# KieDani/UpliftingTableTennis

Measured on AMD Instinct MI355X. Metric: frames/sec end-to-end (detect+uplift), 1280x720, higher is better.
Workload: dtype bf16

## Files before the change

upliftingtabletennis_amd/csrc/conv.hip:

```cpp
#include "conv_mfma.h"
#include "conv64.h"
#include "conv_stem.h"
#include "conv_bneck.h"
#include "conv_bb.h"
#include "chain16.h"
#include "conv_pointwise.h"

namespace ttup {

int launch_stem(const PackedConv& p1, const PackedConv& p2, const PackedConv& p3, const void* x0, void* t2, void* a1,
                int batch, int h, int w, hipStream_t st, int frames_per_sample) {
    TTUP_REQUIRE((p1.cout == 64 && p1.cin_total == 16 && p1.k == 3 && p1.stride == 1 && p1.ck == 16) ||
                 (p1.cout == 64 && p1.cin_total == 128 && p1.k == 1 && p1.ck == 32), TTUP_EINVAL, "stem: unexpected conv1 shape");
    TTUP_REQUIRE(p2.cout == 64 && p2.cin_total == 64 && p2.k == 3 && p2.stride == 1 && p2.ck == 32, TTUP_EINVAL, "stem: unexpected conv2 shape");
    TTUP_REQUIRE(p3.cout == 32 && p3.cin_total == 64 && p3.k == 1 && p3.ck == 32, TTUP_EINVAL, "stem: unexpected follower shape");
    StemArgs a;
    a.x0 = (const bf16_t*)x0; a.w1 = (const bf16_t*)p1.w_dev; a.b1 = p1.bias_dev; a.w2 = (const bf16_t*)p2.w_dev; a.b2 = p2.bias_dev;
    a.w3 = (const bf16_t*)p3.w_dev; a.b3 = p3.bias_dev; a.t2 = (bf16_t*)t2; a.a1 = (bf16_t*)a1;
    a.H = h; a.W = w; a.tiles_x = cdiv(w, 32); a.tiles_per_img = a.tiles_x * cdiv(h, 8); a.total_tiles = a.tiles_per_img * batch;
    constexpr size_t SMEM = (size_t)(5 * 4 * 64 * 8 + 2 * 9 * 4 * 64 * 8 + 2 * 340 * 32 + 432 * 16) * 2;
    static_assert(SMEM <= 160 * 1024, "LDS budget");
    TTUP_REQUIRE(frames_per_sample == 0 || frames_per_sample == 1 || frames_per_sample == 3, TTUP_EINVAL, "stem: frames per sample must be 0 (X0 records), 1 or 3");
    const bool k4 = p1.k == 1;
    TTUP_REQUIRE(k4 == (frames_per_sample == 3), TTUP_EINVAL, "stem: the 4-step conv1 packing is the three-frame form");
// ... 7 lines not shown
                       void* b0, void* b1, int batch, int h, int w, hipStream_t st) {
    TTUP_REQUIRE(p1.cout == 128 && p1.cin_total == 96 && p1.c0 == 32 && p1.k == 1 && p1.ck == 32, TTUP_EINVAL, "bneck_trans: unexpected conv1 shape");
    TTUP_REQUIRE(p5.cout == 16 && p5.cin_total == 128 && p5.k == 3 && p5.stride == 1 && p5.ck == 32, TTUP_EINVAL, "bneck_trans: unexpected conv5 shape");
    TTUP_REQUIRE(p6.cout == 32 && p6.cin_total == 128 && p6.k == 3 && p6.stride == 2 && p6.ck == 32, TTUP_EINVAL, "bneck_trans: unexpected conv6 shape");
    TTUP_REQUIRE(h % 2 == 0 && w % 2 == 0, TTUP_EINVAL, "bneck_trans: even input size required");
    FusedArgs a;
    a.a2 = (const bf16_t*)a2; a.t2 = (const bf16_t*)t2;
    a.w1 = (const bf16_t*)p1.w_dev; a.b1 = p1.bias_dev; a.w5 = (const bf16_t*)p5.w_dev; a.b5 = p5.bias_dev;
    a.w6 = (const bf16_t*)p6.w_dev; a.b6 = p6.bias_dev; a.b0 = (bf16_t*)b0; a.b1o = (bf16_t*)b1;
    a.H = h; a.W = w; a.tiles_x = cdiv(w, 32); a.tiles_per_img = a.tiles_x * cdiv(h, 8); a.total_tiles = a.tiles_per_img * batch;
    constexpr size_t SMEM = (size_t)(340 * 128 + 3 * 8 * 64 * 8 + 4 * 9 * 64 * 8) * 2 + 512;
    return launch_noted(bneck_trans_kernel, dim3(persistent_grid(a.total_tiles)), 512, SMEM, st, a, "bneck_trans_kernel");
}

constexpr int BB2_TH = 24, BB2_TW = 32;
int bb_chain_tiles_per_img(int h, int w) { return cdiv(w, BB2_TW) * cdiv(h, BB2_TH); }

int launch_bb_chain(const PackedConv* const* convs, int n_convs, const void* x, void* y, int batch, int h, int w,
                    const PackedConv* follow, void* y_follow, hipStream_t st, const BBSum* sum) {
    TTUP_REQUIRE(n_convs == 2 || n_convs == 4, TTUP_EINVAL, "bb_chain: 2 or 4 convs expected");
    const int c = convs[0]->cout;
    BBArgs a;
    a.x = (const bf16_t*)x; a.y = (bf16_t*)y;
    if (sum) {
        TTUP_REQUIRE(c == 16 && n_convs == 4 && sum->n_terms >= 0 && sum->n_terms <= 3, TTUP_EINVAL, "bb_chain: the fused fuse-layer sum rides on the 16-channel two-block chain");
        TTUP_REQUIRE(sum->ysum || (sum->heat && sum->head_w && sum->pv && sum->pi), TTUP_EINVAL, "bb_chain: fused sum needs an output");
        a.nsum = sum->n_terms; a.ysum = (bf16_t*)sum->ysum;
        for (int k = 0; k < sum->n_terms; ++k) { a.st[k] = (const bf16_t*)sum->terms[k]; a.ssh[k] = sum->shifts[k]; }
        a.heat = sum->heat; a.hw = sum->head_w; a.hbias = sum->head_bias; a.pv = sum->pv; a.pi = sum->pi;
    }
    if (follow) {
        TTUP_REQUIRE(c == 32 && n_convs == 2 && follow->cout == 16 && follow->cin_total == 32 && follow->k == 1 && follow->ck == 32 && y_follow, TTUP_EINVAL,
                     "bb_chain: the fused follower is a 1x1 32->16 conv on a 32-channel block");
        a.wf = (const bf16_t*)follow->w_dev; a.bf = follow->bias_dev; a.yf = (bf16_t*)y_follow;
    }
    for (int i = 0; i < n_convs; ++i) {
        const PackedConv& p = *convs[i];
        TTUP_REQUIRE(p.cout == c && p.cin_total == c && p.k == 3 && p.stride == 1 && p.ck == (c == 16 ? 16 : 32), TTUP_EINVAL, "bb_chain: unexpected conv shape");
        a.w[i] = (const bf16_t*)p.w_dev; a.bias[i] = p.bias_dev;
    }
    if (c == 16 && n_convs == 4) {
        static const bool generic = env_set("TTUP_BB2_GENERIC");
        bool shifts_ok = true;
        for (int k = 0; k < a.nsum && k < 3; ++k) shifts_ok = shifts_ok && a.ssh[k] == k + 1;
        const bool sum_stored = !generic && shifts_ok && a.nsum >= 1 && a.nsum <= 3 && a.ysum && !a.heat;
        const bool tail = !generic && shifts_ok && a.nsum == 3 && a.heat && !a.y && !a.ysum;
// ... 54 lines not shown
    std::vector<bf16_t> w((size_t)nchunk * ksteps * mt * 64 * 8);
    size_t idx = 0;
    for (int c = 0; c < nchunk; ++c)
        for (int s = 0; s < ksteps; ++s)
            for (int m = 0; m < mt; ++m)
                for (int l = 0; l < 64; ++l) {
                    const int i = l & 15, g = l >> 4;
                    const int co = (i >> 2) * (4 * mt) + m * 4 + (i & 3);
                    for (int j = 0; j < 8; ++j) {
                        int tap, ci;
                        if (ck == 32) { tap = s; ci = c * 32 + 8 * g + j; }
                        else { tap = 2 * s + (g >> 1); ci = c * 16 + 8 * (g & 1) + j; }
                        w[idx++] = f32_to_bf16(tap < taps ? wval(co, ci, tap) : 0.f);
                    }
                }
    out->ck = ck;
    out->w_bytes = w.size() * sizeof(bf16_t);
    TTUP_HIP_CHECK(hipMalloc(&out->w_dev, out->w_bytes));
    TTUP_HIP_CHECK(hipMemcpy(out->w_dev, w.data(), out->w_bytes, hipMemcpyHostToDevice));
    return TTUP_OK;
}

int launch_conv(const PackedConv& p, const ConvLaunch& l, int dtype, hipStream_t st) {
    if (dtype == TTUP_DTYPE_F32) {
        TTUP_REQUIRE(!l.res2 && !l.res3, TTUP_EINVAL, "conv: extra fuse-layer terms are a bf16-path fusion");
        static const bool direct = env_set("TTUP_F32_DIRECT");
        static const bool exact = env_set("TTUP_F32_EXACT");
        if (!direct && !exact && conv_x3_supported(p)) return launch_conv_x3(p, l, st);
        if (!direct && conv_f32_mfma_supported(p)) return launch_conv_f32_mfma(p, l, st);
        TTUP_REQUIRE(!l.n_active, TTUP_EINVAL, "conv: a device-side batch needs the matrix-pipe fp32 kernel");
        ConvFArgs a;
        a.src0 = (const float*)l.src0; a.src1 = (const float*)l.src1; a.w = (const float*)p.w_dev; a.bias = p.bias_dev;
        a.residual = (const float*)l.residual; a.dst = (float*)l.dst;
        a.c0 = p.c0; a.c1 = p.cin_total - p.c0; a.cout = p.cout; a.ks = p.k; a.stride = p.stride;
        a.H = l.h; a.W = l.w; a.OH = (l.h + p.stride - 1) / p.stride; a.OW = (l.w + p.stride - 1) / p.stride; a.relu = l.relu;
        a.total = (long long)l.batch * a.OH * a.OW * a.cout;
        const int threads = 256;
        const long long blocks = (a.total + threads - 1) / threads;
        kernel_note("conv_direct_f32_kernel");
        hipLaunchKernelGGL(conv_direct_f32_kernel, dim3((unsigned)blocks), dim3(threads), 0, st, a);
        TTUP_LAUNCH_CHECK();
        return TTUP_OK;
    }
    TTUP_REQUIRE(!(l.res2 || l.res3) || (p.stride == 2 && !l.follow), TTUP_EINVAL, "conv: extra fuse-layer terms ride on the stride-2 chain convs only");
    if (l.follow) {
        TTUP_REQUIRE(p.k == 3 && p.stride == 1 && p.ck == 32 && p.cout == 64, TTUP_EINVAL, "conv: fused follower needs a 3x3 s1 conv with 64 outputs");
// ... 112 lines not shown
```

upliftingtabletennis_amd/csrc/conv64.h:

```cpp
#pragma once
#include "conv_mfma.h"

namespace ttup {

struct NoHook { __device__ __forceinline__ void operator()(int) const {} };
template <int NPIX = 340, typename Hook = NoHook>
__device__ __forceinline__ void conv64_tile_mfma(f32x4 (&acc)[4][2], const bf16_t* const (&bB)[3], const bf16_t* s_w, int wave, int lane, Hook hook = Hook()) {
    constexpr int IW = 34;
    bf16x8 brow[2][4], af[2][4];
    auto load_b = [&](bf16x8 (&br)[4], int c, int dx) __attribute__((always_inline)) {
#pragma unroll
        for (int rr = 0; rr < 4; ++rr) br[rr] = *(const bf16x8*)(bB[dx] + c * (NPIX * 32) + ((2 * (wave >> 1) + rr) * IW + (wave & 1) * 16) * 32);
    };
    auto load_a = [&](bf16x8 (&a4)[4], int st) __attribute__((always_inline)) {
#pragma unroll
        for (int m = 0; m < 4; ++m) a4[m] = *(const bf16x8*)(s_w + ((st * 4 + m) * 64 + lane) * 8);
    };
    load_b(brow[0], 0, 0);
    load_a(af[0], 0);
#pragma unroll
    for (int s = 0; s < 18; ++s) {
        const int dy = s % 3, gi = s / 3;
        if (s + 1 < 18) {
            const int s1 = s + 1, dy1 = s1 % 3, g1 = s1 / 3, c1 = g1 / 3, dx1 = g1 % 3;
// ... 113 lines not shown
#pragma unroll
                for (int r = 0; r < 4; ++r) v[m * 4 + r] = acc[m][t][r];
            if (a.residual) {
#pragma unroll
                for (int q = 0; q < 2; ++q) {
                    const u32x4 rv = rres[t][q];
                    const unsigned w4[4] = {rv.x, rv.y, rv.z, rv.w};
#pragma unroll
                    for (int k = 0; k < 4; ++k) { v[q * 8 + 2 * k] += bf16_to_f32((bf16_t)(w4[k] & 0xffff)); v[q * 8 + 2 * k + 1] += bf16_to_f32((bf16_t)(w4[k] >> 16)); }
                }
            }
#pragma unroll
            for (int q = 0; q < 2; ++q)
#pragma unroll
                for (int i = 0; i < 4; ++i) { const unsigned w = pack2(v[q * 8 + 2 * i], v[q * 8 + 2 * i + 1]); pk[t][q][i] = a.relu ? relu_pk(w) : w; }
        }
#pragma unroll
        for (int t = 0; t < 2; ++t) {
            const int oy = oy0 + 2 * (wave >> 1) + t, ox = ox0 + (wave & 1) * 16 + n;
            const bool ok = oy < a.H && ox < a.W;
            if (!(L16 || L32) && !ok) continue;
            const size_t opix = ok ? (size_t)(b * a.H + oy) * a.W + ox : 0;
            const size_t o = opix * 64 + g * 16;
#pragma unroll
            for (int q = 0; q < 2; ++q)
                if (ok) *(u32x4*)(a.dst + o + q * 8) = pk[t][q];
            if (L16) {
                f32x4 c = bl16;
#pragma unroll
                for (int k = 0; k < 2; ++k) c = __builtin_amdgcn_mfma_f32_16x16x32_bf16(al16[k], __builtin_bit_cast(bf16x8, pk[t][k]), c, 0, 0, 0);
                if (ok) *(u32x2*)(a.dl16 + opix * 16 + g * 4) = u32x2{pack2(c[0], c[1]), pack2(c[2], c[3])};
            }
            if (L32) {
                f32x4 c[2] = {bl32[0], bl32[1]};
#pragma unroll
                for (int k = 0; k < 2; ++k)
#pragma unroll
                    for (int m = 0; m < 2; ++m) c[m] = __builtin_amdgcn_mfma_f32_16x16x32_bf16(al32[k][m], __builtin_bit_cast(bf16x8, pk[t][k]), c[m], 0, 0, 0);
                if (ok) *(u32x4*)(a.dl32 + opix * 32 + g * 8) = u32x4{pack2(c[0][0], c[0][1]), pack2(c[0][2], c[0][3]), pack2(c[1][0], c[1][1]), pack2(c[1][2], c[1][3])};
            }
        }
    }
}

template <bool L16, bool L32>
__global__ __launch_bounds__(512) void conv64_dma_kernel(ConvKArgs a) {
    constexpr int IH = 10, IW = 34, NPIX = IH * IW;
    constexpr int W_U = 2 * 9 * 4 * 64;
    constexpr int IN_UNITS = NPIX * 8, IN_PT = (IN_UNITS + 511) / 512;
// ... 87 lines not shown
#pragma unroll
                for (int r = 0; r < 4; ++r) v[m * 4 + r] = acc[m][t][r];
            if (a.residual) {
#pragma unroll
                for (int q = 0; q < 2; ++q) {
                    const u32x4 rv = rres[t][q];
                    const unsigned w4[4] = {rv.x, rv.y, rv.z, rv.w};
#pragma unroll
                    for (int k = 0; k < 4; ++k) { v[q * 8 + 2 * k] += bf16_to_f32((bf16_t)(w4[k] & 0xffff)); v[q * 8 + 2 * k + 1] += bf16_to_f32((bf16_t)(w4[k] >> 16)); }
                }
            }
#pragma unroll
            for (int q = 0; q < 2; ++q)
#pragma unroll
                for (int i = 0; i < 4; ++i) { const unsigned w = pack2(v[q * 8 + 2 * i], v[q * 8 + 2 * i + 1]); pk[t][q][i] = a.relu ? relu_pk(w) : w; }
        }
#pragma unroll
        for (int t = 0; t < 2; ++t) {
            const int oy = oy0 + 2 * (wave >> 1) + t, ox = ox0 + (wave & 1) * 16 + n;
            const bool ok = oy < a.H && ox < a.W;
            if (!(L16 || L32) && !ok) continue;
            const size_t opix = ok ? (size_t)(b * a.H + oy) * a.W + ox : 0;
            const size_t o = opix * 64 + g * 16;
#pragma unroll
            for (int q = 0; q < 2; ++q)
                if (ok) *(u32x4*)(a.dst + o + q * 8) = pk[t][q];
            if (L16) {
                f32x4 c = bl16;
#pragma unroll
                for (int k = 0; k < 2; ++k) c = __builtin_amdgcn_mfma_f32_16x16x32_bf16(al16[k], __builtin_bit_cast(bf16x8, pk[t][k]), c, 0, 0, 0);
                if (ok) *(u32x2*)(a.dl16 + opix * 16 + g * 4) = u32x2{pack2(c[0], c[1]), pack2(c[2], c[3])};
            }
            if (L32) {
                f32x4 c[2] = {bl32[0], bl32[1]};
#pragma unroll
                for (int k = 0; k < 2; ++k)
#pragma unroll
                    for (int m = 0; m < 2; ++m) c[m] = __builtin_amdgcn_mfma_f32_16x16x32_bf16(al32[k][m], __builtin_bit_cast(bf16x8, pk[t][k]), c[m], 0, 0, 0);
                if (ok) *(u32x4*)(a.dl32 + opix * 32 + g * 8) = u32x4{pack2(c[0][0], c[0][1]), pack2(c[0][2], c[0][3]), pack2(c[1][0], c[1][1]), pack2(c[1][2], c[1][3])};
            }
        }
    };
    f32x4 acc[4][2];
    u32x4 rres[2][2] = {};
    for (int it = 0; it < my_tiles; ++it) {
        const TileAt tile = tile_at<8, 32>(xcd_tile(blockIdx.x + it * gridDim.x, a.total_tiles), a.tiles_per_img, a.tiles_x);
        const int b = tile.b, oy0 = tile.y0, ox0 = tile.x0;
        __syncthreads();
        if (a.residual) {
// ... 18 lines not shown
        epilogue(acc, rres, b, oy0, ox0);
    }
}

template <bool DMA, bool L16, bool L32>
static int launch_conv64_t(const ConvKArgs& a, hipStream_t st) {
    constexpr size_t SMEM = (size_t)(2 * 9 * 4 * 64 * 8 + (DMA ? 2 : 1) * 2 * 340 * 32) * 2;
    return launch_noted(DMA ? conv64_dma_kernel<L16, L32> : conv64_kernel<L16, L32>, dim3(persistent_grid(a.total_tiles)), 512, SMEM, st, a,
                        DMA ? "conv64_dma_kernel<%s, %s>" : "conv64_kernel<%s, %s>", L16 ? "true" : "false", L32 ? "true" : "false");
}
template <bool DMA>
static int launch_conv64_followers(const ConvKArgs& a, hipStream_t st) {
    if (a.dl16 && a.dl32) return launch_conv64_t<DMA, true, true>(a, st);
    if (a.dl16) return launch_conv64_t<DMA, true, false>(a, st);
    if (a.dl32) return launch_conv64_t<DMA, false, true>(a, st);
    return launch_conv64_t<DMA, false, false>(a, st);
}

static int launch_conv64(const PackedConv& p, const ConvLaunch& l, hipStream_t st) {
    ConvKArgs a;
    a.src0 = (const bf16_t*)l.src0; a.wpack = (const bf16_t*)p.w_dev; a.bias = p.bias_dev; a.residual = (const bf16_t*)l.residual; a.dst = (bf16_t*)l.dst;
    a.H = l.h; a.W = l.w; a.OH = l.h; a.OW = l.w; a.relu = l.relu;
    a.tiles_x = cdiv(l.w, 32); a.tiles_per_img = a.tiles_x * cdiv(l.h, 8); a.total_tiles = a.tiles_per_img * l.batch;
    if (l.lin16) {
        TTUP_REQUIRE(l.lin16->cout == 16 && l.lin16->cin_total == 64 && l.lin16->k == 1 && l.lin16->ck == 32 && l.lin16_dst, TTUP_EINVAL, "conv64: bad 64->16 follower");
        a.wl16 = (const bf16_t*)l.lin16->w_dev; a.bl16 = l.lin16->bias_dev; a.dl16 = (bf16_t*)l.lin16_dst;
    }
    if (l.lin32) {
        TTUP_REQUIRE(l.lin32->cout == 32 && l.lin32->cin_total == 64 && l.lin32->k == 1 && l.lin32->ck == 32 && l.lin32_dst, TTUP_EINVAL, "conv64: bad 64->32 follower");
        a.wl32 = (const bf16_t*)l.lin32->w_dev; a.bl32 = l.lin32->bias_dev; a.dl32 = (bf16_t*)l.lin32_dst;
    }
    static const bool dma = env_ll("TTUP_CONV64_DMA", 1) != 0;
    return dma ? launch_conv64_followers<true>(a, st) : launch_conv64_followers<false>(a, st);
}

}
```

upliftingtabletennis_amd/csrc/conv_mfma.h:

```cpp
#pragma once
#include "conv_dev.h"
#include "conv.h"

namespace ttup {

struct ConvKArgs {
    const bf16_t* src0 = nullptr;
    const bf16_t* src1 = nullptr;
    const bf16_t* wpack = nullptr;
    const float* bias = nullptr;
    const bf16_t* residual = nullptr;
    bf16_t* dst = nullptr;
    int c0 = 0, c1 = 0;
    int nchunk0 = 0, nchunk = 0;
    int H = 0, W = 0, OH = 0, OW = 0;
    int tiles_x = 0, tiles_per_img = 0, total_tiles = 0;
    int relu = 0;
    const bf16_t* w11 = nullptr; const float* bias11 = nullptr; bf16_t* dst11 = nullptr;
    const bf16_t* res2 = nullptr; const bf16_t* res3 = nullptr; int sh3 = 0;
    const bf16_t* wl16 = nullptr; const float* bl16 = nullptr; bf16_t* dl16 = nullptr;
    const bf16_t* wl32 = nullptr; const float* bl32 = nullptr; bf16_t* dl32 = nullptr;
    const bf16_t* wpack_b = nullptr; const float* bias_b = nullptr; bf16_t* dst_b = nullptr; int relu_b = 0;
    int xcd = 0;
};
// ... 211 lines not shown
                    *(u32x4*)(s_t + p * 64 + (((2 * g + q) ^ (p & 7)) << 3)) = pk;
                }
            }
            __syncthreads();
#pragma unroll
            for (int t = 0; t < NT; ++t) {
                const int nt = wave * NT + t;
                const int p = (nt / NTW) * TW + (nt % NTW) * 16 + n;
                f32x4 c11[2] = {bias11[0], bias11[1]};
#pragma unroll
                for (int k = 0; k < 2; ++k) {
                    const bf16x8 bfr = *(const bf16x8*)(s_t + p * 64 + (((4 * k + g) ^ (p & 7)) << 3));
#pragma unroll
                    for (int m = 0; m < 2; ++m) c11[m] = __builtin_amdgcn_mfma_f32_16x16x32_bf16(af11[k][m], bfr, c11[m], 0, 0, 0);
                }
                const int oy = oy0 + nt / NTW, ox = ox0 + (nt % NTW) * 16 + n;
                if (oy >= a.OH || ox >= a.OW) continue;
                *(u32x4*)(a.dst11 + ((size_t)(b * a.OH + oy) * a.OW + ox) * 32 + g * 8) = pack8(c11[0], c11[1], true);
            }
        }
    }
}

__global__ __launch_bounds__(512) void conv_s2_pair_kernel(ConvKArgs a) {
    constexpr int CK = 16, KS = 3, S = 2, TH = 4, TW = 32, MTA = 2, MTB = 1;
    constexpr int IH = (TH - 1) * S + KS, IW = (TW - 1) * S + KS;
    constexpr int KSTEPS = 5, PAD = 1;
    constexpr int IN_ELEMS = IH * IW * CK;
    constexpr int IN_UNITS = IH * IW * (CK / 8), IN_PT = (IN_UNITS + 511) / 512;
    constexpr int WA_UNITS = KSTEPS * MTA * 64, WB_UNITS = KSTEPS * MTB * 64;
    extern __shared__ __attribute__((aligned(16))) char smem[];
    bf16_t* s_in = (bf16_t*)smem;
    bf16_t* s_wa = s_in + ((IN_ELEMS + 7) & ~7);
    bf16_t* s_wb = s_wa + WA_UNITS * 8;
    const int tid = threadIdx.x, lane = tid & 63, wave = __builtin_amdgcn_readfirstlane(tid >> 6);
    const int n = lane & 15, g = lane >> 4;
    const int my_tiles = (a.total_tiles - (int)blockIdx.x + (int)gridDim.x - 1) / (int)gridDim.x;
    StageRegs<WA_UNITS> wa; StageRegs<WB_UNITS> wb;
    stage_load_512<WA_UNITS>(wa, a.wpack, tid);
    stage_load_512<WB_UNITS>(wb, a.wpack_b, tid);
    u32x4 pin[IN_PT];
    unsigned pin_ok = 0u;
    auto issue = [&](int it) {
        const TileAt t = tile_at<TH * S, TW * S, PAD>(xcd_tile(blockIdx.x + it * gridDim.x, a.total_tiles), a.tiles_per_img, a.tiles_x);
        const int b = t.b, gy0 = t.y0, gx0 = t.x0;
#pragma unroll
        for (int k = 0; k < IN_PT; ++k) {
            const int u = tid + k * 512;
            const int c8 = u % (CK / 8), pix = u / (CK / 8);
            const int gy = gy0 + pix / IW, gx = gx0 + pix % IW;
            const bool ok = u < IN_UNITS && gy >= 0 && gy < a.H && gx >= 0 && gx < a.W;
            pin[k] = *(const u32x4*)(ok ? a.src0 + ((size_t)(b * a.H + gy) * a.W + gx) * CK + c8 * 8 : a.src0);
            pin_ok = ok ? pin_ok | (1u << k) : pin_ok & ~(1u << k);
        }
    };
    if (my_tiles <= 0) return;
    issue(0);
    stage_store_512<WA_UNITS>(s_wa, wa, tid);
    stage_store_512<WB_UNITS>(s_wb, wb, tid);
    f32x4 bias_a[MTA], bias_b;
#pragma unroll
    for (int m = 0; m < MTA; ++m) bias_a[m] = *(const f32x4*)(a.bias + g * 4 * MTA + m * 4);
    bias_b = *(const f32x4*)(a.bias_b + g * 4);
    const bf16_t* bB[KSTEPS];
#pragma unroll
    for (int k = 0; k < KSTEPS; ++k) {
        int tap = 2 * k + (g >> 1);
        if (tap > 8) tap = 8;
        bB[k] = s_in + lds_off<CK, IW>(tap / KS, n * S + tap % KS, g & 1);
    }
    const int r = wave >> 1, cg = wave & 1;
    prefetch_arrived(pin);
    for (int it = 0; it < my_tiles; ++it) {
        if (it > 0) __syncthreads();
#pragma unroll
        for (int k = 0; k < IN_PT; ++k) {
            const int u = tid + k * 512;
            const bool okk = (pin_ok >> k) & 1u;
            if (u < IN_UNITS) { const int c8 = u % (CK / 8), pix = u / (CK / 8); *(u32x4*)(s_in + lds_off<CK, IW>(pix / IW, pix % IW, c8)) = u32x4{okk ? pin[k].x : 0u, okk ? pin[k].y : 0u, okk ? pin[k].z : 0u, okk ? pin[k].w : 0u}; }
        }
        __syncthreads();
        if (it + 1 < my_tiles) issue(it + 1);
        f32x4 acc_a[MTA] = {bias_a[0], bias_a[1]}, acc_b = bias_b;
#pragma unroll
        for (int s5 = 0; s5 < KSTEPS; ++s5) {
            const bf16x8 bfr = *(const bf16x8*)(bB[s5] + ((r * S) * IW + cg * 16 * S) * CK);
#pragma unroll
            for (int m = 0; m < MTA; ++m) acc_a[m] = __builtin_amdgcn_mfma_f32_16x16x32_bf16(*(const bf16x8*)(s_wa + ((s5 * MTA + m) * 64 + lane) * 8), bfr, acc_a[m], 0, 0, 0);
            acc_b = __builtin_amdgcn_mfma_f32_16x16x32_bf16(*(const bf16x8*)(s_wb + (s5 * 64 + lane) * 8), bfr, acc_b, 0, 0, 0);
        }
        prefetch_arrived(pin);
        const int tl = xcd_tile(blockIdx.x + it * gridDim.x, a.total_tiles);
        const int b = tl / a.tiles_per_img, tt = tl % a.tiles_per_img;
        const int oy = (tt / a.tiles_x) * TH + r, ox = (tt % a.tiles_x) * TW + cg * 16 + n;
        if (oy >= a.OH || ox >= a.OW) continue;
        const size_t opix = (size_t)(b * a.OH + oy) * a.OW + ox;
        {
            const size_t o = opix * 32 + g * 8;
            float v[8];
#pragma unroll
            for (int m = 0; m < MTA; ++m)
#pragma unroll
                for (int q = 0; q < 4; ++q) v[m * 4 + q] = acc_a[m][q];
            auto add_term = [&](const bf16_t* base) { add_bf16x8(v, *(const u32x4*)base); };
            if (a.residual) add_term(a.residual + o);
            if (a.res2) add_term(a.res2 + o);
            if (a.res3) add_term(a.res3 + ((size_t)(b * (a.OH >> a.sh3) + (oy >> a.sh3)) * (a.OW >> a.sh3) + (ox >> a.sh3)) * 32 + g * 8);
            *(u32x4*)(a.dst + o) = pack8(v, a.relu);
        }
        {
            const unsigned w0 = pack2(acc_b[0], acc_b[1]), w1 = pack2(acc_b[2], acc_b[3]);
            *(u32x2*)(a.dst_b + opix * 16 + g * 4) = u32x2{a.relu_b ? relu_pk(w0) : w0, a.relu_b ? relu_pk(w1) : w1};
        }
    }
}

template <int CK, int COUT, int KS, int S, int TH, int TW, int NW, bool F11 = false>
static int launch_mfma(const PackedConv& p, const ConvLaunch& l, hipStream_t st) {
    constexpr int MT = COUT / 16;
    constexpr int IH = (TH - 1) * S + KS, IW = (TW - 1) * S + KS;
    constexpr int KSTEPS = (CK == 32) ? KS * KS : (KS * KS + 1) / 2;
    constexpr size_t SMEM = (size_t)(((IH * IW * CK + 7) & ~7) + KSTEPS * MT * 64 * 8) * 2;
    static_assert(SMEM <= 160 * 1024, "LDS budget");
    ConvKArgs a;
    a.src0 = (const bf16_t*)l.src0; a.src1 = (const bf16_t*)l.src1; a.wpack = (const bf16_t*)p.w_dev; a.bias = p.bias_dev;
    a.residual = (const bf16_t*)l.residual; a.dst = (bf16_t*)l.dst;
    a.c0 = p.c0; a.c1 = p.cin_total - p.c0; a.nchunk0 = p.c0 / CK; a.nchunk = p.cin_total / CK;
    a.H = l.h; a.W = l.w; a.OH = (l.h + S - 1) / S; a.OW = (l.w + S - 1) / S;
    a.tiles_x = cdiv(a.OW, TW); a.tiles_per_img = a.tiles_x * cdiv(a.OH, TH); a.total_tiles = a.tiles_per_img * l.batch;
    a.relu = l.relu;
    a.res2 = (const bf16_t*)l.res2; a.res3 = (const bf16_t*)l.res3; a.sh3 = l.sh3;
    if (F11) {
        TTUP_REQUIRE(l.follow && l.follow->cout == 32 && l.follow->cin_total == 64 && l.follow->k == 1 && l.follow->ck == 32 && l.dst2, TTUP_EINVAL, "conv: bad fused 1x1 follower");
        a.w11 = (const bf16_t*)l.follow->w_dev; a.bias11 = l.follow->bias_dev; a.dst11 = (bf16_t*)l.dst2;
    }
    static const int s2_xcd = (int)env_ll("TTUP_S2_XCD", 0);
    a.xcd = (S == 2) ? s2_xcd : 0;
    const int per_cu = (int)((160 * 1024) / SMEM) > 4 ? 4 : ((int)((160 * 1024) / SMEM) < 1 ? 1 : (int)((160 * 1024) / SMEM));
    return launch_noted(conv_mfma_kernel<CK, COUT, KS, S, TH, TW, NW, F11>, dim3(persistent_grid(a.total_tiles, per_cu)), NW * 64, SMEM, st, a,
                        "conv_mfma_kernel<%d, %d, %d, %d, %d, %d, %d, %s>", CK, COUT, KS, S, TH, TW, NW, F11 ? "true" : "false");
}

static int launch_s2_pair(const PackedConv& p, const ConvLaunch& l, hipStream_t st) {
    const PackedConv& q = *l.pair;
    TTUP_REQUIRE(p.k == 3 && p.stride == 2 && p.ck == 16 && p.cin_total == 16 && p.cout == 32 && q.k == 3 && q.stride == 2 && q.ck == 16 &&
                 q.cin_total == 16 && q.cout == 16 && l.pair_dst && !l.src1, TTUP_EINVAL, "conv: the paired form is 3x3 s2 16 -> 32 with 3x3 s2 16 -> 16");
    ConvKArgs a;
    a.src0 = (const bf16_t*)l.src0; a.wpack = (const bf16_t*)p.w_dev; a.bias = p.bias_dev; a.residual = (const bf16_t*)l.residual; a.dst = (bf16_t*)l.dst;
    a.res2 = (const bf16_t*)l.res2; a.res3 = (const bf16_t*)l.res3; a.sh3 = l.sh3; a.relu = l.relu;
    a.wpack_b = (const bf16_t*)q.w_dev; a.bias_b = q.bias_dev; a.dst_b = (bf16_t*)l.pair_dst; a.relu_b = l.pair_relu;
    a.H = l.h; a.W = l.w; a.OH = (l.h + 1) / 2; a.OW = (l.w + 1) / 2;
    a.tiles_x = cdiv(a.OW, 32); a.tiles_per_img = a.tiles_x * cdiv(a.OH, 4); a.total_tiles = a.tiles_per_img * l.batch;
    constexpr size_t SMEM = (size_t)(((9 * 65 * 16 + 7) & ~7) + 5 * 3 * 64 * 8) * 2;
    return launch_noted(conv_s2_pair_kernel, dim3(persistent_grid(a.total_tiles, 4)), 512, SMEM, st, a, "conv_s2_pair_kernel");
}

template <int CK, int KS, int S, int TH, int TW>
static int dispatch_cout(const PackedConv& p, const ConvLaunch& l, hipStream_t st) {
    if constexpr (CK == 32 && S == 2) {
        if (p.cout == 64) return launch_mfma<CK, 64, KS, S, TH, TW, 4>(p, l, st);
    }
    switch (p.cout) {
        case 16: return launch_mfma<CK, 16, KS, S, TH, TW, 8>(p, l, st);
        case 32: return launch_mfma<CK, 32, KS, S, TH, TW, 8>(p, l, st);
        case 64: return launch_mfma<CK, 64, KS, S, TH, TW, 8>(p, l, st);
        case 128: return launch_mfma<CK, 128, KS, S, TH, TW, 8>(p, l, st);
    }
    set_error("conv: cout %d unsupported", p.cout);
    return TTUP_EINVAL;
}

}
```

upliftingtabletennis_amd/csrc/wasb_net.h:

```cpp
#pragma once
#include "conv.h"

namespace ttup {
size_t upsum_head_ws_bytes(int n_maps, int H, int W);
int launch_upsum_head(const void* base, const void* const* terms, const int* shifts, int n_terms, const float* w_dev, float bias,
                      float* heat, int n_maps, int H, int W, long long* argmax, float* win, void* ws, size_t ws_bytes, hipStream_t st);
int refine_argmax(const float* heat, int n_maps, int H, int W, long long* argmax, float* win, void* ws, size_t ws_bytes, hipStream_t st);
int launch_argmax_finish(const float* heat, int n_maps, int H, int W, int nblk, const float* pv, const long long* pi, long long* argmax, float* win, hipStream_t st);

struct Tensor : TensorShape { void* ptr = nullptr; };

struct CertState {
    bool enabled = false;
    float eps = 0.f;
    static constexpr float GUARD = 1.25f;
    int R = CERT_R;
    int small = 0;
    int K = 256;
    int maxc = 8;
    int maxf = 8;
    int CH = 0, nchunks = 0, max_crops = 0, Hc = 0, Wc = 0;
    int budget = 0;
    bool exact_windows = false;
    int audit_mod = 0, audit_phase = 0;
// ... 4 lines not shown
        int* guard_cnt = nullptr;
        int* status = nullptr; int* n_crops = nullptr;
        int* cand_idx = nullptr; int* cand_crop = nullptr; float* cand_val = nullptr; float* cand_win = nullptr;
        float* cand_bf = nullptr;
        CropRec* crop_rec = nullptr; int* n_active = nullptr;
        int* roi_flag = nullptr;
        float* margin = nullptr;
        hipEvent_t done = nullptr;
        hipEvent_t read_status = nullptr, read_info = nullptr, read_margin = nullptr;
    } slot[2];
    int cur = 0;
    unsigned long long* stats = nullptr;
    float* crop_heat = nullptr;
    hipStream_t stream = nullptr;
    hipEvent_t lanes_done = nullptr;
};
}

struct ttup_wasb {
    int H = 0, W = 0, max_batch = 0, dtype = 0, micro = 1, in_ch = 9;
    std::vector<ttup::PackedConv> convs;
    std::vector<ttup::Tensor> tensors;
    std::vector<ttup::Op> ops;
    std::map<std::string, int> taps;
    int t_input = -1, t_out = -1;
    int t_frames = -1;
    bool frames_mode = false;
    float* head_w_dev = nullptr; float* head_b_dev = nullptr; float head_bias = 0.f;
    int n_out = 1;
    float* heat_scratch = nullptr;
    void* refine_ws = nullptr; size_t refine_ws_bytes = 0;
    long long* argmax_scratch = nullptr; float* win_scratch = nullptr;
    int last_batch = 0;
    bool fused_head = false;
    const int* n_active = nullptr;
    std::vector<ttup::Roi> op_roi; ttup::Roi out_roi; const int* roi_flag = nullptr;
    std::vector<char> blob;
    ttup::CertState cert;
    struct Lane {
        std::vector<void*> ptr;
        float* heat_scratch = nullptr; void* refine_ws = nullptr; long long* argmax_scratch = nullptr; float* win_scratch = nullptr;
        hipStream_t stream = nullptr; hipEvent_t done = nullptr;
    };
    std::vector<Lane> lanes;
    hipEvent_t fork = nullptr;
    hipEvent_t pass_done = nullptr;
// ... 21 lines not shown
```

upliftingtabletennis_amd/csrc/wasb_net.hip:

```cpp
#include "wasb_net.h"
#include "wasb_blob.h"
#include <string.h>
#include <stdlib.h>
#include <memory>

using namespace ttup;

ttup_wasb::~ttup_wasb() {
    cert_free(this);
    for (auto& c : convs) free_conv(&c);
    for (auto& L : lanes) {
        for (void* q : L.ptr) if (q) (void)hipFree(q);
        if (L.heat_scratch) (void)hipFree(L.heat_scratch);
        if (L.refine_ws) (void)hipFree(L.refine_ws);
        if (L.argmax_scratch) (void)hipFree(L.argmax_scratch);
        if (L.win_scratch) (void)hipFree(L.win_scratch);
        if (L.stream) (void)hipStreamDestroy(L.stream);
        if (L.done) (void)hipEventDestroy(L.done);
    }
    if (fork) (void)hipEventDestroy(fork);
    if (pass_done) (void)hipEventDestroy(pass_done);
    if (head_w_dev) (void)hipFree(head_w_dev);
    if (head_b_dev) (void)hipFree(head_b_dev);
}

namespace {

void chain_args(const ttup_wasb* net, const Op& op, const PackedConv* cv[4], BBSum* sum) {
    for (int k = 0; k < 4; ++k) cv[k] = k < op.n_chain ? &net->convs[op.chain[k]] : nullptr;
    sum->n_terms = op.n_terms;
    for (int k = 0; k < op.n_terms; ++k) { sum->terms[k] = net->tensors[op.terms[k]].ptr; sum->shifts[k] = op.shifts[k]; }
}

int run_op(ttup_wasb* net, const Op& op, int mb, hipStream_t st) {
    if (op.kind == Op::CONV) {
        const Tensor& s = net->tensors[op.src0];
        ConvLaunch l;
        l.src0 = s.ptr; l.src1 = op.src1 >= 0 ? net->tensors[op.src1].ptr : nullptr;
        l.residual = op.residual >= 0 ? net->tensors[op.residual].ptr : nullptr;
        l.dst = net->tensors[op.dst].ptr; l.batch = mb; l.h = s.h; l.w = s.w; l.relu = op.relu; l.n_active = net->n_active;
        if (!net->op_roi.empty() && net->roi_flag) { l.roi = net->op_roi[&op - net->ops.data()]; l.roi.flag = net->roi_flag; }
        if (op.conv2 >= 0) { l.follow = &net->convs[op.conv2]; l.dst2 = net->tensors[op.dst2].ptr; }
        if (op.lin16 >= 0) { l.lin16 = &net->convs[op.lin16]; l.lin16_dst = net->tensors[op.lin16_dst].ptr; }
        if (op.lin32 >= 0) { l.lin32 = &net->convs[op.lin32]; l.lin32_dst = net->tensors[op.lin32_dst].ptr; }
        if (op.pair >= 0) { l.pair = &net->convs[op.pair]; l.pair_dst = net->tensors[op.pair_dst].ptr; l.pair_relu = op.pair_relu; }
        if (op.res2 >= 0) l.res2 = net->tensors[op.res2].ptr;
        if (op.res3 >= 0) { l.res3 = net->tensors[op.res3].ptr; l.sh3 = op.sh3; }
        const int rc = launch_conv(net->convs[op.conv], l, net->dtype, st);
        if (rc) return rc;
    } else if (op.kind == Op::STEM) {
        const Tensor& s = net->tensors[op.src0];
        const bool fm = net->frames_mode && net->t_frames >= 0 && op.conv1f >= 0;
        const int rc = launch_stem(net->convs[fm ? op.conv1f : op.conv], net->convs[op.conv2], net->convs[op.conv3], fm ? net->tensors[net->t_frames].ptr : s.ptr,
                                   net->tensors[op.dst].ptr, net->tensors[op.dst2].ptr, mb, s.h, s.w, st, fm ? net->in_ch / 3 : 0);
        if (rc) return rc;
    } else if (op.kind == Op::UPSUM_HEAD) {
        return TTUP_OK;
    } else if (op.kind == Op::BB_CHAIN) {
        if (op.head) return TTUP_OK;
        const Tensor& s = net->tensors[op.src0];
        const PackedConv* cv[4]; BBSum sum;
        chain_args(net, op, cv, &sum);
        int rc;
        if (op.n_chain == 4 && op.n_terms > 0) {
            sum.ysum = net->tensors[op.dst2].ptr;
            rc = launch_bb_chain(cv, 4, s.ptr, op.dst >= 0 ? net->tensors[op.dst].ptr : nullptr, mb, s.h, s.w, nullptr, nullptr, st, &sum);
        } else {
            rc = launch_bb_chain(cv, op.n_chain, s.ptr, net->tensors[op.dst].ptr, mb, s.h, s.w,
                                 op.conv2 >= 0 ? &net->convs[op.conv2] : nullptr, op.dst2 >= 0 ? net->tensors[op.dst2].ptr : nullptr, st);
        }
        if (rc) return rc;
    } else if (op.kind == Op::BNECK_TRANS) {
        const Tensor& s = net->tensors[op.src0];
        const int rc = launch_bneck_trans(net->convs[op.conv], net->convs[op.conv2], net->convs[op.conv3], s.ptr, net->tensors[op.src1].ptr,
                                          net->tensors[op.dst].ptr, net->tensors[op.dst2].ptr, mb, s.h, s.w, st);
        if (rc) return rc;
    } else {
        const Tensor& d = net->tensors[op.dst];
        const void* terms[3] = {nullptr, nullptr, nullptr};
        for (int k = 0; k < op.n_terms; ++k) terms[k] = net->tensors[op.terms[k]].ptr;
        Roi roi;
        if (!net->op_roi.empty() && net->roi_flag) { roi = net->op_roi[&op - net->ops.data()]; roi.flag = net->roi_flag; }
        const int rc = launch_upsum(net->tensors[op.src0].ptr, terms, op.shifts, op.n_terms, d.ptr, mb, d.h, d.w, d.c, net->dtype, st, net->n_active, &roi);
        if (rc) return rc;
    }
    return TTUP_OK;
}

int run_graph(ttup_wasb* net, int mb, hipStream_t st) {
    for (const Op& op : net->ops) { const int rc = run_op(net, op, mb, st); if (rc) return rc; }
    return TTUP_OK;
// ... 174 lines not shown
    TTUP_REQUIRE(max_batch > 0, TTUP_EINVAL, "ttup_wasb_create: max_batch must be positive");
    TTUP_REQUIRE(dtype == TTUP_DTYPE_BF16 || dtype == TTUP_DTYPE_F32, TTUP_EINVAL, "ttup_wasb_create: unknown dtype %d", dtype);
    std::vector<FoldedConv> folded;
    std::vector<float> head_w, head_b;
    int in_ch = 0, head_out = 0;
    int rc = parse_blob(blob, blob_bytes, &folded, &in_ch, &head_out, &head_w, &head_b);
    if (rc) return rc;
    TTUP_REQUIRE((in_ch == 9 || in_ch == 3) && head_out >= 1 && head_out <= 16, TTUP_EFORMAT, "wasb blob: in_ch=%d head_out=%d unsupported (ball detector 9/3, table detector 3/13)", in_ch, head_out);
    int ndev = 0;
    TTUP_HIP_CHECK(hipGetDeviceCount(&ndev));
    TTUP_REQUIRE(ndev > 0, TTUP_EHIP, "ttup_wasb_create: no HIP device");
    std::unique_ptr<ttup_wasb> net(new ttup_wasb);
    net->H = height; net->W = width; net->max_batch = max_batch; net->dtype = dtype; net->in_ch = in_ch;
    net->blob.assign((const char*)blob, (const char*)blob + blob_bytes);
    net->n_out = head_out == 3 ? 1 : head_out;
    int micro = micro_override > 0 ? micro_override : (int)env_ll("TTUP_MICRO_BATCH", 8);
    if (micro < 1) micro = 1;
    net->micro = micro < max_batch ? micro : max_batch;
    GraphSwitches sw;
    sw.fuse = !env_set("TTUP_NO_FUSE"); sw.fuse_sum = !env_set("TTUP_NO_FUSE_SUM"); sw.fuse_lin = !env_set("TTUP_NO_FUSE_LIN");
    sw.pair = !env_set("TTUP_NO_PAIR"); sw.stem = !env_set("TTUP_NO_STEM"); sw.frames_mode = !env_set("TTUP_NO_FRAMES_MODE");
    const GraphPlan plan = build_graph(folded, in_ch, net->n_out, height, width, net->micro, dtype, sw);
    if (plan.rc) return plan.rc;
    net->ops = plan.ops; net->taps = plan.taps;
    net->t_input = plan.t_input; net->t_out = plan.t_out; net->t_frames = plan.t_frames; net->fused_head = plan.fused_head;
    for (const TensorShape& s : plan.tensors) { Tensor t; static_cast<TensorShape&>(t) = s; net->tensors.push_back(t); }
    for (const ConvRequest& r : plan.convs) {
        net->convs.emplace_back();
        PackedConv& p = net->convs.back();
        rc = pack_conv(plan.source_a(r, folded), r.b >= 0 ? &folded[r.b] : nullptr, r.cin_pad, dtype, &p);
        if (rc) return rc;
        TTUP_REQUIRE(p.cout == r.cout && p.cin_total == r.cin_total && p.c0 == r.c0 && p.k == r.k && p.stride == r.stride, TTUP_EINVAL,
                     "wasb: conv %zu was packed as %d x %d+%d, k %d / s%d; the plan has %d x %d+%d, k %d / s%d", net->convs.size() - 1,
                     p.cout, p.c0, p.cin_total - p.c0, p.k, p.stride, r.cout, r.c0, r.cin_total - r.c0, r.k, r.stride);
    }
    {
        const int first = head_out == 3 ? 1 : 0;
        TTUP_HIP_CHECK(hipMalloc((void**)&net->head_w_dev, (size_t)net->n_out * 16 * sizeof(float)));
        TTUP_HIP_CHECK(hipMemcpy(net->head_w_dev, head_w.data() + (size_t)first * 16, (size_t)net->n_out * 16 * sizeof(float), hipMemcpyHostToDevice));
        TTUP_HIP_CHECK(hipMalloc((void**)&net->head_b_dev, (size_t)net->n_out * sizeof(float)));
        TTUP_HIP_CHECK(hipMemcpy(net->head_b_dev, head_b.data() + first, (size_t)net->n_out * sizeof(float), hipMemcpyHostToDevice));
        net->head_bias = head_b[first];
    }
    const size_t hw = (size_t)height * width;
    net->refine_ws_bytes = ttup_refine_workspace_bytes(net->micro * net->n_out, height, width);
    if (upsum_head_ws_bytes(net->micro, height, width) > net->refine_ws_bytes) net->refine_ws_bytes = upsum_head_ws_bytes(net->micro, height, width);
    {
// ... 124 lines not shown
```

Before: 2209.

## Skip dead conv outputs beside fused followers; prefetch pair-kernel residual terms

Adds a reader analysis over the graph plan and passes a null destination when a conv's main output feeds only a fused 1x1 follower and nothing else reads it. The 64-channel and bb-chain kernels then skip that global store, which cuts write bandwidth. The stride-2 pair kernel now keeps its bias in LDS instead of registers, loads the res2/res3 terms before the MFMA loop so their latency overlaps compute, and sets launch bounds with a minimum of 6 blocks. The risks are register pressure from the early loads and the correctness of the reader analysis.

```diff
diff --git a/upliftingtabletennis_amd/csrc/conv.hip b/upliftingtabletennis_amd/csrc/conv.hip
--- a/upliftingtabletennis_amd/csrc/conv.hip
+++ b/upliftingtabletennis_amd/csrc/conv.hip
@@ -53,6 +53,7 @@
     const int c = convs[0]->cout;
     BBArgs a;
     a.x = (const bf16_t*)x; a.y = (bf16_t*)y;
+    TTUP_REQUIRE(y || (follow && y_follow) || sum, TTUP_EINVAL, "bb_chain: no output tensor");
     if (sum) {
         TTUP_REQUIRE(c == 16 && n_convs == 4 && sum->n_terms >= 0 && sum->n_terms <= 3, TTUP_EINVAL, "bb_chain: the fused fuse-layer sum rides on the 16-channel two-block chain");
         TTUP_REQUIRE(sum->ysum || (sum->heat && sum->head_w && sum->pv && sum->pi), TTUP_EINVAL, "bb_chain: fused sum needs an output");
@@ -153,6 +154,7 @@
 }
 
 int launch_conv(const PackedConv& p, const ConvLaunch& l, int dtype, hipStream_t st) {
+    TTUP_REQUIRE(l.dst || (dtype == TTUP_DTYPE_BF16 && (l.lin16 || l.lin32) && !l.follow && !l.pair), TTUP_EINVAL, "conv: no output tensor");
     if (dtype == TTUP_DTYPE_F32) {
         TTUP_REQUIRE(!l.res2 && !l.res3, TTUP_EINVAL, "conv: extra fuse-layer terms are a bf16-path fusion");
         static const bool direct = env_set("TTUP_F32_DIRECT");
diff --git a/upliftingtabletennis_amd/csrc/conv64.h b/upliftingtabletennis_amd/csrc/conv64.h
--- a/upliftingtabletennis_amd/csrc/conv64.h
+++ b/upliftingtabletennis_amd/csrc/conv64.h
@@ -159,9 +159,11 @@
             if (!(L16 || L32) && !ok) continue;
             const size_t opix = ok ? (size_t)(b * a.H + oy) * a.W + ox : 0;
             const size_t o = opix * 64 + g * 16;
-#pragma unroll
-            for (int q = 0; q < 2; ++q)
-                if (ok) *(u32x4*)(a.dst + o + q * 8) = pk[t][q];
+            if (a.dst) {
+#pragma unroll
+                for (int q = 0; q < 2; ++q)
+                    if (ok) *(u32x4*)(a.dst + o + q * 8) = pk[t][q];
+            }
             if (L16) {
                 f32x4 c = bl16;
 #pragma unroll
@@ -295,9 +297,11 @@
             if (!(L16 || L32) && !ok) continue;
             const size_t opix = ok ? (size_t)(b * a.H + oy) * a.W + ox : 0;
             const size_t o = opix * 64 + g * 16;
-#pragma unroll
-            for (int q = 0; q < 2; ++q)
-                if (ok) *(u32x4*)(a.dst + o + q * 8) = pk[t][q];
+            if (a.dst) {
+#pragma unroll
+                for (int q = 0; q < 2; ++q)
+                    if (ok) *(u32x4*)(a.dst + o + q * 8) = pk[t][q];
+            }
             if (L16) {
                 f32x4 c = bl16;
 #pragma unroll
@@ -362,6 +366,7 @@
     a.src0 = (const bf16_t*)l.src0; a.wpack = (const bf16_t*)p.w_dev; a.bias = p.bias_dev; a.residual = (const bf16_t*)l.residual; a.dst = (bf16_t*)l.dst;
     a.H = l.h; a.W = l.w; a.OH = l.h; a.OW = l.w; a.relu = l.relu;
     a.tiles_x = cdiv(l.w, 32); a.tiles_per_img = a.tiles_x * cdiv(l.h, 8); a.total_tiles = a.tiles_per_img * l.batch;
+    TTUP_REQUIRE(l.dst || l.lin16 || l.lin32, TTUP_EINVAL, "conv64: no output -- the 64-channel store may only be left out beside a follower");
     if (l.lin16) {
         TTUP_REQUIRE(l.lin16->cout == 16 && l.lin16->cin_total == 64 && l.lin16->k == 1 && l.lin16->ck == 32 && l.lin16_dst, TTUP_EINVAL, "conv64: bad 64->16 follower");
         a.wl16 = (const bf16_t*)l.lin16->w_dev; a.bl16 = l.lin16->bias_dev; a.dl16 = (bf16_t*)l.lin16_dst;
diff --git a/upliftingtabletennis_amd/csrc/conv_mfma.h b/upliftingtabletennis_amd/csrc/conv_mfma.h
--- a/upliftingtabletennis_amd/csrc/conv_mfma.h
+++ b/upliftingtabletennis_amd/csrc/conv_mfma.h
@@ -257,7 +257,7 @@
     }
 }
 
-__global__ __launch_bounds__(512) void conv_s2_pair_kernel(ConvKArgs a) {
+__global__ __launch_bounds__(512, 6) void conv_s2_pair_kernel(ConvKArgs a) {
     constexpr int CK = 16, KS = 3, S = 2, TH = 4, TW = 32, MTA = 2, MTB = 1;
     constexpr int IH = (TH - 1) * S + KS, IW = (TW - 1) * S + KS;
     constexpr int KSTEPS = 5, PAD = 1;
@@ -268,6 +268,7 @@
     bf16_t* s_in = (bf16_t*)smem;
     bf16_t* s_wa = s_in + ((IN_ELEMS + 7) & ~7);
     bf16_t* s_wb = s_wa + WA_UNITS * 8;
+    float* s_bias = (float*)(s_wb + WB_UNITS * 8);
     const int tid = threadIdx.x, lane = tid & 63, wave = __builtin_amdgcn_readfirstlane(tid >> 6);
     const int n = lane & 15, g = lane >> 4;
     const int my_tiles = (a.total_tiles - (int)blockIdx.x + (int)gridDim.x - 1) / (int)gridDim.x;
@@ -293,10 +294,8 @@
     issue(0);
     stage_store_512<WA_UNITS>(s_wa, wa, tid);
     stage_store_512<WB_UNITS>(s_wb, wb, tid);
-    f32x4 bias_a[MTA], bias_b;
-#pragma unroll
-    for (int m = 0; m < MTA; ++m) bias_a[m] = *(const f32x4*)(a.bias + g * 4 * MTA + m * 4);
-    bias_b = *(const f32x4*)(a.bias_b + g * 4);
+    if (tid < 32) s_bias[tid] = a.bias[tid];
+    else if (tid < 48) s_bias[tid] = a.bias_b[tid - 32];
     const bf16_t* bB[KSTEPS];
 #pragma unroll
     for (int k = 0; k < KSTEPS; ++k) {
@@ -316,20 +315,27 @@
         }
         __syncthreads();
         if (it + 1 < my_tiles) issue(it + 1);
-        f32x4 acc_a[MTA] = {bias_a[0], bias_a[1]}, acc_b = bias_b;
-#pragma unroll
-        for (int s5 = 0; s5 < KSTEPS; ++s5) {
-            const bf16x8 bfr = *(const bf16x8*)(bB[s5] + ((r * S) * IW + cg * 16 * S) * CK);
-#pragma unroll
-            for (int m = 0; m < MTA; ++m) acc_a[m] = __builtin_amdgcn_mfma_f32_16x16x32_bf16(*(const bf16x8*)(s_wa + ((s5 * MTA + m) * 64 + lane) * 8), bfr, acc_a[m], 0, 0, 0);
-            acc_b = __builtin_amdgcn_mfma_f32_16x16x32_bf16(*(const bf16x8*)(s_wb + (s5 * 64 + lane) * 8), bfr, acc_b, 0, 0, 0);
-        }
-        prefetch_arrived(pin);
         const int tl = xcd_tile(blockIdx.x + it * gridDim.x, a.total_tiles);
         const int b = tl / a.tiles_per_img, tt = tl % a.tiles_per_img;
         const int oy = (tt / a.tiles_x) * TH + r, ox = (tt % a.tiles_x) * TW + cg * 16 + n;
-        if (oy >= a.OH || ox >= a.OW) continue;
+        const bool live = oy < a.OH && ox < a.OW;
         const size_t opix = (size_t)(b * a.OH + oy) * a.OW + ox;
+        u32x4 term[2];
+        {
+            const size_t o3 = ((size_t)(b * (a.OH >> a.sh3) + (oy >> a.sh3)) * (a.OW >> a.sh3) + (ox >> a.sh3)) * 32 + g * 8;
+            term[0] = *(const u32x4*)(a.res2 && live ? a.res2 + opix * 32 + g * 8 : a.src0);
+            term[1] = *(const u32x4*)(a.res3 && live ? a.res3 + o3 : a.src0);
+        }
+        f32x4 acc_a[MTA] = {*(const f32x4*)(s_bias + g * 4 * MTA), *(const f32x4*)(s_bias + g * 4 * MTA + 4)}, acc_b = *(const f32x4*)(s_bias + 32 + g * 4);
+#pragma unroll
+        for (int s5 = 0; s5 < KSTEPS; ++s5) {
+            const bf16x8 bfr = *(const bf16x8*)(bB[s5] + ((r * S) * IW + cg * 16 * S) * CK);
+#pragma unroll
+            for (int m = 0; m < MTA; ++m) acc_a[m] = __builtin_amdgcn_mfma_f32_16x16x32_bf16(*(const bf16x8*)(s_wa + ((s5 * MTA + m) * 64 + lane) * 8), bfr, acc_a[m], 0, 0, 0);
+            acc_b = __builtin_amdgcn_mfma_f32_16x16x32_bf16(*(const bf16x8*)(s_wb + (s5 * 64 + lane) * 8), bfr, acc_b, 0, 0, 0);
+        }
+        prefetch_arrived(pin); prefetch_arrived(term);
+        if (!live) continue;
         {
             const size_t o = opix * 32 + g * 8;
             float v[8];
@@ -337,10 +343,9 @@
             for (int m = 0; m < MTA; ++m)
 #pragma unroll
                 for (int q = 0; q < 4; ++q) v[m * 4 + q] = acc_a[m][q];
-            auto add_term = [&](const bf16_t* base) { add_bf16x8(v, *(const u32x4*)base); };
-            if (a.residual) add_term(a.residual + o);
-            if (a.res2) add_term(a.res2 + o);
-            if (a.res3) add_term(a.res3 + ((size_t)(b * (a.OH >> a.sh3) + (oy >> a.sh3)) * (a.OW >> a.sh3) + (ox >> a.sh3)) * 32 + g * 8);
+            if (a.residual) add_bf16x8(v, *(const u32x4*)(a.residual + o));
+            if (a.res2) add_bf16x8(v, term[0]);
+            if (a.res3) add_bf16x8(v, term[1]);
             *(u32x4*)(a.dst + o) = pack8(v, a.relu);
         }
         {
@@ -386,7 +391,8 @@
     a.wpack_b = (const bf16_t*)q.w_dev; a.bias_b = q.bias_dev; a.dst_b = (bf16_t*)l.pair_dst; a.relu_b = l.pair_relu;
     a.H = l.h; a.W = l.w; a.OH = (l.h + 1) / 2; a.OW = (l.w + 1) / 2;
     a.tiles_x = cdiv(a.OW, 32); a.tiles_per_img = a.tiles_x * cdiv(a.OH, 4); a.total_tiles = a.tiles_per_img * l.batch;
-    constexpr size_t SMEM = (size_t)(((9 * 65 * 16 + 7) & ~7) + 5 * 3 * 64 * 8) * 2;
+    constexpr size_t PAIR_BIAS_BYTES = (32 + 16) * sizeof(float);
+    constexpr size_t SMEM = (size_t)(((9 * 65 * 16 + 7) & ~7) + 5 * 3 * 64 * 8) * 2 + PAIR_BIAS_BYTES;
     return launch_noted(conv_s2_pair_kernel, dim3(persistent_grid(a.total_tiles, 4)), 512, SMEM, st, a, "conv_s2_pair_kernel");
 }
 
diff --git a/upliftingtabletennis_amd/csrc/wasb_net.h b/upliftingtabletennis_amd/csrc/wasb_net.h
--- a/upliftingtabletennis_amd/csrc/wasb_net.h
+++ b/upliftingtabletennis_amd/csrc/wasb_net.h
@@ -50,6 +50,7 @@
     std::vector<ttup::PackedConv> convs;
     std::vector<ttup::Tensor> tensors;
     std::vector<ttup::Op> ops;
+    std::vector<char> has_reader;
     std::map<std::string, int> taps;
     int t_input = -1, t_out = -1;
     int t_frames = -1;
diff --git a/upliftingtabletennis_amd/csrc/wasb_net.hip b/upliftingtabletennis_amd/csrc/wasb_net.hip
--- a/upliftingtabletennis_amd/csrc/wasb_net.hip
+++ b/upliftingtabletennis_amd/csrc/wasb_net.hip
@@ -1,5 +1,6 @@
 #include "wasb_net.h"
 #include "wasb_blob.h"
+#include "wasb_readers.h"
 #include <string.h>
 #include <stdlib.h>
 #include <memory>
@@ -32,13 +33,18 @@
     for (int k = 0; k < op.n_terms; ++k) { sum->terms[k] = net->tensors[op.terms[k]].ptr; sum->shifts[k] = op.shifts[k]; }
 }
 
+void* stored_dst(const ttup_wasb* net, const Op& op, bool has_follower) {
+    if (op.dst < 0) return nullptr;
+    return has_follower && !net->has_reader[op.dst] ? nullptr : net->tensors[op.dst].ptr;
+}
+
 int run_op(ttup_wasb* net, const Op& op, int mb, hipStream_t st) {
     if (op.kind == Op::CONV) {
         const Tensor& s = net->tensors[op.src0];
         ConvLaunch l;
         l.src0 = s.ptr; l.src1 = op.src1 >= 0 ? net->tensors[op.src1].ptr : nullptr;
         l.residual = op.residual >= 0 ? net->tensors[op.residual].ptr : nullptr;
-        l.dst = net->tensors[op.dst].ptr; l.batch = mb; l.h = s.h; l.w = s.w; l.relu = op.relu; l.n_active = net->n_active;
+        l.dst = stored_dst(net, op, net->dtype == TTUP_DTYPE_BF16 && op.conv2 < 0 && op.pair < 0 && (op.lin16 >= 0 || op.lin32 >= 0)); l.batch = mb; l.h = s.h; l.w = s.w; l.relu = op.relu; l.n_active = net->n_active;
         if (!net->op_roi.empty() && net->roi_flag) { l.roi = net->op_roi[&op - net->ops.data()]; l.roi.flag = net->roi_flag; }
         if (op.conv2 >= 0) { l.follow = &net->convs[op.conv2]; l.dst2 = net->tensors[op.dst2].ptr; }
         if (op.lin16 >= 0) { l.lin16 = &net->convs[op.lin16]; l.lin16_dst = net->tensors[op.lin16_dst].ptr; }
@@ -66,7 +72,7 @@
             sum.ysum = net->tensors[op.dst2].ptr;
             rc = launch_bb_chain(cv, 4, s.ptr, op.dst >= 0 ? net->tensors[op.dst].ptr : nullptr, mb, s.h, s.w, nullptr, nullptr, st, &sum);
         } else {
-            rc = launch_bb_chain(cv, op.n_chain, s.ptr, net->tensors[op.dst].ptr, mb, s.h, s.w,
+            rc = launch_bb_chain(cv, op.n_chain, s.ptr, stored_dst(net, op, op.n_chain == 2 && op.conv2 >= 0 && op.dst2 >= 0), mb, s.h, s.w,
                                  op.conv2 >= 0 ? &net->convs[op.conv2] : nullptr, op.dst2 >= 0 ? net->tensors[op.dst2].ptr : nullptr, st);
         }
         if (rc) return rc;
@@ -287,7 +293,7 @@
     sw.pair = !env_set("TTUP_NO_PAIR"); sw.stem = !env_set("TTUP_NO_STEM"); sw.frames_mode = !env_set("TTUP_NO_FRAMES_MODE");
     const GraphPlan plan = build_graph(folded, in_ch, net->n_out, height, width, net->micro, dtype, sw);
     if (plan.rc) return plan.rc;
-    net->ops = plan.ops; net->taps = plan.taps;
+    net->ops = plan.ops; net->taps = plan.taps; net->has_reader = tensor_readers(plan);
     net->t_input = plan.t_input; net->t_out = plan.t_out; net->t_frames = plan.t_frames; net->fused_head = plan.fused_head;
     for (const TensorShape& s : plan.tensors) { Tensor t; static_cast<TensorShape&>(t) = s; net->tensors.push_back(t); }
     for (const ConvRequest& r : plan.convs) {
diff --git a/upliftingtabletennis_amd/csrc/wasb_readers.h b/upliftingtabletennis_amd/csrc/wasb_readers.h
--- /dev/null
+++ b/upliftingtabletennis_amd/csrc/wasb_readers.h
@@ -0,0 +1,18 @@
+#pragma once
+#include "wasb_graph.h"
+
+namespace ttup {
+
+inline std::vector<char> tensor_readers(const GraphPlan& g) {
+    std::vector<char> read(g.tensors.size(), 0);
+    auto mark = [&](int t) { if (t >= 0 && t < (int)read.size()) read[t] = 1; };
+    for (const Op& op : g.ops) {
+        mark(op.src0); mark(op.src1); mark(op.residual); mark(op.res2); mark(op.res3);
+        for (int k = 0; k < op.n_terms && k < 3; ++k) mark(op.terms[k]);
+    }
+    for (const auto& kv : g.taps) mark(kv.second);
+    mark(g.t_input); mark(g.t_frames); mark(g.t_out);
+    return read;
+}
+
+}
```

New measurement: 2215, median of 6. No clear change (+0.3%).
